# hyllios/CGAT

Measured on AMD Instinct MI355X. Metric: edges/sec through one CGAT attention layer (fwd+bwd), 1M-edge batch, higher is better.
Workload: dtype f32 storage / f16x3c (24-bit operands: exact h + l + t split, 3 fp16 + 3 six-bit matrix passes where built, six bf16 passes elsewhere; fp32 accumulate); 1 GPU; one GATConvNodes layer (H_Net update) fwd+bwd, 4167 crystals x 20 atoms x 12 nbrs per rank: N=83340, E=1000080, C=Ce=128, H=3, scalar attention; edges_per_rank=1000080, parallelism=dp1 (graphs sharded, gradient all-reduce)

## Files before the change

### cgat_amd/csrc/rowsdw.hip

```cpp
#include <string.h>

#include "common.h"
#include "kernels.h"
#include "mfma_bf16.h"

typedef float f32x16 __attribute__((ext_vector_type(16)));

template <int NX>
__device__ __forceinline__ void rows_dw128_body(const float* __restrict__ G, long ldg, const float* __restrict__ X1,
                                                long ldx1, const float* __restrict__ X2, long ldx2,
                                                float* __restrict__ o, int nbeg, int nend, float* red) {
  constexpr int U = 4;
  const int tid = threadIdx.x, lane = tid & 63, wave = tid >> 6;
  const int w = wave & 3, h = wave >> 2;
  const int l32 = lane & 31, hi = lane >> 5;
  const int nbatch = (nend - nbeg + 4 * U - 1) / (4 * U);

  f32x16 acc[NX][4];
#pragma unroll
  for (int k = 0; k < NX; ++k)
#pragma unroll
    for (int j = 0; j < 4; ++j)
#pragma unroll
      for (int t = 0; t < 16; ++t) acc[k][j][t] = 0.f;
  float cs = 0.f;

  float ga[3][U];
  float4 xa[3][U], xb[3][NX > 1 ? U : 1];
#define DW_LOAD(buf_, b_)                                                                     \
  {                                                                                           \
    _Pragma("unroll") for (int u = 0; u < U; ++u) {                                           \
      const int row = nbeg + 2 * U * (2 * (b_) + h) + 2 * u + hi;                             \
      const bool ok = row < nend;                                                             \
      const long rr = ok ? row : nbeg;                                                        \
      const float g = G[rr * ldg + 4 * l32 + w];                                              \
      const float4 x = *reinterpret_cast<const float4*>(X1 + rr * ldx1 + 4 * l32);            \
      ga[buf_][u] = ok ? g : 0.f;                                                             \
      xa[buf_][u] = x;                                                                        \
      if constexpr (NX > 1) xb[buf_][u] = *reinterpret_cast<const float4*>(X2 + rr * ldx2 + 4 * l32); \
    }                                                                                         \
  }
#define DW_MFMA(buf_)                                                                         \
  {                                                                                           \
    _Pragma("unroll") for (int u = 0; u < U; ++u) {                                           \
      const float a = ga[buf_][u];                                                            \
      cs += a;                                                                                \
      acc[0][0] = __builtin_amdgcn_mfma_f32_32x32x2f32(a, xa[buf_][u].x, acc[0][0], 0, 0, 0); \
      acc[0][1] = __builtin_amdgcn_mfma_f32_32x32x2f32(a, xa[buf_][u].y, acc[0][1], 0, 0, 0); \
      acc[0][2] = __builtin_amdgcn_mfma_f32_32x32x2f32(a, xa[buf_][u].z, acc[0][2], 0, 0, 0); \
      acc[0][3] = __builtin_amdgcn_mfma_f32_32x32x2f32(a, xa[buf_][u].w, acc[0][3], 0, 0, 0); \
      if constexpr (NX > 1) {                                                                 \
        acc[NX - 1][0] = __builtin_amdgcn_mfma_f32_32x32x2f32(a, xb[buf_][u].x, acc[NX - 1][0], 0, 0, 0); \
        acc[NX - 1][1] = __builtin_amdgcn_mfma_f32_32x32x2f32(a, xb[buf_][u].y, acc[NX - 1][1], 0, 0, 0); \
        acc[NX - 1][2] = __builtin_amdgcn_mfma_f32_32x32x2f32(a, xb[buf_][u].z, acc[NX - 1][2], 0, 0, 0); \
        acc[NX - 1][3] = __builtin_amdgcn_mfma_f32_32x32x2f32(a, xb[buf_][u].w, acc[NX - 1][3], 0, 0, 0); \
      }                                                                                       \
    }                                                                                         \
  }
  DW_LOAD(0, 0);
  DW_LOAD(1, 1);
  for (int b = 0; b < nbatch; b += 3) {
    DW_LOAD(2, b + 2);
    DW_MFMA(0);
    if (b + 1 < nbatch) {
      DW_LOAD(0, b + 3);
      DW_MFMA(1);
    }
    if (b + 2 < nbatch) {
      DW_LOAD(1, b + 4);
      DW_MFMA(2);
    }
  }
#undef DW_LOAD
#undef DW_MFMA
  cs += __shfl_xor(cs, 32);
  if (h == 1) {
#pragma unroll
    for (int k = 0; k < NX; ++k)
#pragma unroll
      for (int t = 0; t < 16; ++t) {
        const int m = (t & 3) + 8 * (t >> 2) + 4 * hi;
        *reinterpret_cast<float4*>(&red[(k * 128 + 4 * m + w) * 128 + 4 * l32]) =
            make_float4(acc[k][0][t], acc[k][1][t], acc[k][2][t], acc[k][3][t]);
      }
    if (hi == 0) red[NX * 128 * 128 + 4 * l32 + w] = cs;
  }
  __syncthreads();
  if (h == 0) {
#pragma unroll
    for (int k = 0; k < NX; ++k)
#pragma unroll
      for (int t = 0; t < 16; ++t) {
        const int m = (t & 3) + 8 * (t >> 2) + 4 * hi;
        const int idx = (k * 128 + 4 * m + w) * 128 + 4 * l32;
        const float4 r = *reinterpret_cast<const float4*>(&red[idx]);
        *reinterpret_cast<float4*>(o + idx) =
            make_float4(acc[k][0][t] + r.x, acc[k][1][t] + r.y, acc[k][2][t] + r.z, acc[k][3][t] + r.w);
      }
    if (hi == 0) o[NX * 128 * 128 + 4 * l32 + w] = cs + red[NX * 128 * 128 + 4 * l32 + w];
  }
}

template <int NX>
__global__ __launch_bounds__(512, 1) void rows_dw128_kernel(const float* __restrict__ G, long ldg,
                                                            const float* __restrict__ X1, long ldx1,
                                                            const float* __restrict__ X2, long ldx2,
                                                            float* __restrict__ slab, int rows, int rows_per_wg) {
  constexpr int SLAB = NX * 128 * 128 + 128;
  extern __shared__ float red[];
  const int nbeg = blockIdx.x * rows_per_wg;
  rows_dw128_body<NX>(G, ldg, X1, ldx1, X2, ldx2, slab + (long)blockIdx.x * SLAB, nbeg, min(rows, nbeg + rows_per_wg), red);
}

__global__ __launch_bounds__(512, 1) void rows_dw128_batch_kernel(DwBatchDesc d, float* __restrict__ slab) {
  extern __shared__ float red[];
  const int item = blockIdx.x / d.splits, sp = blockIdx.x - item * d.splits;
  const float* G = d.it[item].G;
  const float* X = d.it[item].X;
  const int nbeg = sp * d.rows_per_unit;
  rows_dw128_body<1>(G, d.ldg, X, d.ldx, X, d.ldx, slab + (long)blockIdx.x * (16384 + 128), nbeg,
                     min(d.rows, nbeg + d.rows_per_unit), red);
}
#define DWS_PITCH 80
#define DWS_IMG (128 * DWS_PITCH)
__global__ __launch_bounds__(512, 1) void rows_dw128_split_batch_kernel(DwBatchDesc d, float* __restrict__ slab) {
  extern __shared__ __attribute__((aligned(16))) unsigned char lds[];
  const int item = blockIdx.x / d.splits, sp = blockIdx.x - item * d.splits;
  const float* G = d.it[item].G;
  const float* X = d.it[item].X;
  const int nbeg = sp * d.rows_per_unit, nend = min(d.rows, nbeg + d.rows_per_unit);
  float* o = slab + (long)blockIdx.x * (16384 + 128);
  const int tid = threadIdx.x, lane = tid & 63, wave = tid >> 6;
  const int opnd = tid >> 8, m = tid & 127, half = (tid >> 7) & 1;
  const float* src = opnd ? X : G;
  const long ld = opnd ? d.ldx : d.ldg;
  unsigned char* wr_base = lds + (size_t)opnd * 3 * DWS_IMG + (size_t)m * DWS_PITCH + half * 32;
  const int wo = wave & 3, wi = wave >> 2;
  const int n16 = lane & 15, kg = lane >> 4;
  const unsigned char* rdA = lds + (size_t)(32 * wo + n16) * DWS_PITCH + kg * 16;
  const unsigned char* rdB = lds + (size_t)3 * DWS_IMG + (size_t)(64 * wi + n16) * DWS_PITCH + kg * 16;

  f32x4 accp[8], accn[8];
#pragma unroll
  for (int i = 0; i < 8; ++i) { accp[i] = f32x4{0.f, 0.f, 0.f, 0.f}; accn[i] = f32x4{0.f, 0.f, 0.f, 0.f}; }
  float cs = 0.f;
  const int nsteps = (nend - nbeg + 31) / 32;

  float va[16], vb[16];
#define DWS_LOAD(V_, s_)                                                                     \
  {                                                                                          \
    _Pragma("unroll") for (int u = 0; u < 16; ++u) {                                         \
      const int row = nbeg + 32 * (s_) + 16 * half + u;                                      \
      const bool ok = row < nend;                                                            \
      const float t = src[(long)(ok ? row : nend - 1) * ld + m];                             \
      V_[u] = (ok || opnd) ? t : 0.f;                                                        \
    }                                                                                        \
  }
#define DWS_STEP(V_, s_, ACC_, NEG_)                                                         \
  {                                                                                          \
    {                                                                                        \
      float w[16];                                                                           \
      _Pragma("unroll") for (int u = 0; u < 16; ++u) {                                       \
        if (!opnd) cs += V_[u];                                                              \
        w[u] = (NEG_ && !opnd) ? -V_[u] : V_[u];                                             \
      }                                                                                      \
      unsigned char* wp = wr_base + (size_t)((s_) & 1) * 6 * DWS_IMG;                        \
      _Pragma("unroll") for (int h8 = 0; h8 < 2; ++h8) {                                     \
        const float v8[8] = {w[8 * h8], w[8 * h8 + 1], w[8 * h8 + 2], w[8 * h8 + 3],         \
                             w[8 * h8 + 4], w[8 * h8 + 5], w[8 * h8 + 6], w[8 * h8 + 7]};    \
        bf16x8 q1, q2, q3;                                                                   \
        split3_x8(v8, q1, q2, q3);                                                           \
        *reinterpret_cast<bf16x8*>(wp + 16 * h8) = q1;                                       \
        *reinterpret_cast<bf16x8*>(wp + DWS_IMG + 16 * h8) = q2;                             \
        *reinterpret_cast<bf16x8*>(wp + 2 * DWS_IMG + 16 * h8) = q3;                         \
      }                                                                                      \
    }                                                                                        \
    DWS_LOAD(V_, (s_) + 2)    \
     \
    asm volatile("s_waitcnt lgkmcnt(0)" ::: "memory");                                       \
    __builtin_amdgcn_s_barrier();                                                            \
    asm volatile("" ::: "memory");                                                           \
    {                                                                                        \
      const unsigned char* pa = rdA + (size_t)((s_) & 1) * 6 * DWS_IMG;                      \
      const unsigned char* pb = rdB + (size_t)((s_) & 1) * 6 * DWS_IMG;                      \
      bf16x8 a1[2], a2[2], a3[2];                                                            \
      _Pragma("unroll") for (int ob = 0; ob < 2; ++ob) {                                     \
        a1[ob] = *reinterpret_cast<const bf16x8*>(pa + (size_t)16 * ob * DWS_PITCH);         \
        a2[ob] = *reinterpret_cast<const bf16x8*>(pa + DWS_IMG + (size_t)16 * ob * DWS_PITCH);      \
        a3[ob] = *reinterpret_cast<const bf16x8*>(pa + 2 * DWS_IMG + (size_t)16 * ob * DWS_PITCH);  \
      }                                                                                      \
      _Pragma("unroll") for (int ib = 0; ib < 4; ++ib) {                                     \
        const bf16x8 b1 = *reinterpret_cast<const bf16x8*>(pb + (size_t)16 * ib * DWS_PITCH);               \
        const bf16x8 b2 = *reinterpret_cast<const bf16x8*>(pb + DWS_IMG + (size_t)16 * ib * DWS_PITCH);     \
        const bf16x8 b3 = *reinterpret_cast<const bf16x8*>(pb + 2 * DWS_IMG + (size_t)16 * ib * DWS_PITCH); \
        _Pragma("unroll") for (int ob = 0; ob < 2; ++ob) {                                   \
          f32x4 c = ACC_[4 * ob + ib];                                                       \
          c = mma16<false>(a3[ob], b1, c);                         \
          c = mma16<false>(a1[ob], b3, c);                                                   \
          c = mma16<false>(a2[ob], b2, c);                                                   \
          c = mma16<false>(a2[ob], b1, c);                                                   \
          c = mma16<false>(a1[ob], b2, c);                                                   \
          c = mma16<false>(a1[ob], b1, c);                                                   \
          ACC_[4 * ob + ib] = c;                                                             \
        }                                                                                    \
      }                                                                                      \
    }                                                                                        \
  }
  DWS_LOAD(va, 0)
  DWS_LOAD(vb, 1)
  for (int s = 0; s < nsteps; s += 2) {
    DWS_STEP(va, s, accp, false)
    DWS_STEP(vb, s + 1, accn, true)
  }
#undef DWS_LOAD
#undef DWS_STEP
#pragma unroll
  for (int ob = 0; ob < 2; ++ob)
#pragma unroll
    for (int ib = 0; ib < 4; ++ib)
#pragma unroll
      for (int t = 0; t < 4; ++t) {
        const int orow = 32 * wo + 16 * ob + 4 * kg + t, icol = 64 * wi + 16 * ib + n16;
        float r = accp[4 * ob + ib][t] - accn[4 * ob + ib][t];
        asm volatile("" : "+v"(r));
        o[orow * 128 + icol] = r;
      }
  __syncthreads();
  float* red = reinterpret_cast<float*>(lds);
  if (!opnd && half == 1) red[m] = cs;
  __syncthreads();
  if (!opnd && half == 0) o[16384 + m] = cs + red[m];
}

__global__ __launch_bounds__(256) void rows_dw128_reduce_batch_kernel(const float* __restrict__ slab, DwBatchDesc d) {
  __shared__ float part[8][32];
  const int item = blockIdx.y;
  const int o = threadIdx.x & 31, zg = threadIdx.x >> 5;
  const long total = 16384 + 128;
  const long i = (long)blockIdx.x * 32 + o;
  const float* sl = slab + (long)item * d.splits * total;
  const int per = (d.splits + 7) / 8;
  const int z0 = zg * per, z1 = min(d.splits, z0 + per);
  float s = 0.f;
  if (i < total)
    for (int z = z0; z < z1; ++z) s += sl[(long)z * total + i];
  part[zg][o] = s;
  __syncthreads();
  if (zg != 0 || i >= total) return;
  s = part[0][o];
#pragma unroll
  for (int g = 1; g < 8; ++g) s += part[g][o];
  if (i < 16384) d.it[item].out[(i >> 7) * d.ldo + (i & 127)] = s;
  else if (d.it[item].bsum) d.it[item].bsum[i - 16384] = s;
}

__global__ __launch_bounds__(256) void rows_dw128_reduce_kernel(const float* __restrict__ slab, int splits, int nx,
                                                                float* __restrict__ out1, long ldo1,
                                                                float* __restrict__ out2, long ldo2,
                                                                float* __restrict__ bsum) {
  __shared__ float part[8][32];
  const int o = threadIdx.x & 31, zg = threadIdx.x >> 5;
  const long total = (long)nx * 16384 + 128, stride = total;
  const long i = (long)blockIdx.x * 32 + o;
  const int per = (splits + 7) / 8;
  const int z0 = zg * per, z1 = min(splits, z0 + per);
  float s = 0.f;
  if (i < total)
    for (int z = z0; z < z1; ++z) s += slab[(long)z * stride + i];
  part[zg][o] = s;
  __syncthreads();
  if (zg != 0 || i >= total) return;
  s = part[0][o];
#pragma unroll
  for (int g = 1; g < 8; ++g) s += part[g][o];
  if (i < 16384) out1[(i >> 7) * ldo1 + (i & 127)] = s;
  else if (nx > 1 && i < 32768) out2[((i - 16384) >> 7) * ldo2 + (i & 127)] = s;
  else if (bsum) bsum[i - (long)nx * 16384] = s;
}

int rows_dw128_batch_launch(DwBatchDesc d, void* ws, size_t ws_bytes, hipStream_t stream);
static int dw_rows_per_wg(int rows) {
  int rps = cdiv(cdiv(rows, 256), 16) * 16;
  return rps < 16 ? 16 : rps;
}
bool rows_dw128_fast(const float* G, long ldg, const float* X1, long ldx1, const float* X2, long ldx2) {
  return (ldg % 4) == 0 && (ldx1 % 4) == 0 && (((uintptr_t)G) & 15) == 0 && (((uintptr_t)X1) & 15) == 0 &&
         (!X2 || ((ldx2 % 4) == 0 && (((uintptr_t)X2) & 15) == 0));
}
size_t rows_dw128_batch_ws_bytes(int n_items, int rows);
size_t rows_dw128_ws_bytes(int rows, int nx) {
  const int splits = cdiv(rows, dw_rows_per_wg(rows));
  size_t b = ws_round((size_t)splits * ((size_t)nx * 16384 + 128), 4);
  if (nx == 1) {
    const size_t c = rows_dw128_batch_ws_bytes(1, rows);
    if (c > b) b = c;
  }
  return b;
}
int rows_dw128_launch(const float* G, long ldg, const float* X1, long ldx1, float* out1, long ldo1, const float* X2,
                      long ldx2, float* out2, long ldo2, float* bsum, int rows, void* ws, size_t ws_bytes,
                      hipStream_t stream) {
  const int nx = X2 ? 2 : 1;
  if (rows <= 0) {
    for (int o = 0; o < 128; ++o) {
      CGAT_TRY(fill_launch(out1 + o * ldo1, 0.f, 128, stream));
      if (X2) CGAT_TRY(fill_launch(out2 + o * ldo2, 0.f, 128, stream));
    }
    if (bsum) CGAT_TRY(fill_launch(bsum, 0.f, 128, stream));
    return CGAT_OK;
  }
  const size_t need = rows_dw128_ws_bytes(rows, nx);
  if (!ws || ws_bytes < need) {
    cgat_set_error("rows_dw128: workspace too small (%zu < %zu)", ws_bytes, need);
    return CGAT_ERR_WORKSPACE;
  }
  if (nx == 1 && mode_split()) {
    DwBatchDesc b;
    memset(&b, 0, sizeof(b));
    b.n = 1; b.rows = rows; b.ldg = ldg; b.ldx = ldx1; b.ldo = ldo1;
    b.it[0] = {G, X1, out1, bsum};
    return rows_dw128_batch_launch(b, ws, ws_bytes, stream);
  }
  const int rps = dw_rows_per_wg(rows), splits = cdiv(rows, rps);
  const size_t lds = ((size_t)nx * 16384 + 128) * sizeof(float);
  {
    CGAT_PROF("rows_dw", stream);
    if (nx == 2) {
      static bool attr = false;
      if (!attr) {
        CGAT_HIP(hipFuncSetAttribute((const void*)rows_dw128_kernel<2>, hipFuncAttributeMaxDynamicSharedMemorySize, (int)lds));
        attr = true;
      }
      hipLaunchKernelGGL(rows_dw128_kernel<2>, dim3(splits), dim3(512), lds, stream, G, ldg, X1, ldx1, X2, ldx2,
                         (float*)ws, rows, rps);
    } else {
      static bool attr = false;
      if (!attr) {
        CGAT_HIP(hipFuncSetAttribute((const void*)rows_dw128_kernel<1>, hipFuncAttributeMaxDynamicSharedMemorySize, (int)lds));
        attr = true;
      }
      hipLaunchKernelGGL(rows_dw128_kernel<1>, dim3(splits), dim3(512), lds, stream, G, ldg, X1, ldx1, X1, ldx1,
                         (float*)ws, rows, rps);
    }
    CGAT_LAUNCH_CHECK();
  }
  const long total = (long)nx * 16384 + 128;
  hipLaunchKernelGGL(rows_dw128_reduce_kernel, dim3(cdiv(total, 32)), dim3(256), 0, stream, (const float*)ws, splits, nx,
                     out1, ldo1, out2, ldo2, bsum);
  CGAT_LAUNCH_CHECK();
  return CGAT_OK;
}

static int dw_batch_splits(int n_items, int rows) {
  int sp = 256 / (n_items > 0 ? n_items : 1);
  const int most = cdiv(rows, 64);
  if (sp > most) sp = most;
  return sp < 1 ? 1 : sp;
}
size_t rows_dw128_batch_ws_bytes(int n_items, int rows) {
  if (n_items < 1) n_items = 1;
  const long most = cdiv(rows > 0 ? rows : 1, 64);
  long units = n_items > 256 ? n_items : 256;
  if (units > (long)n_items * most) units = (long)n_items * most;
  return ws_round((size_t)units * (16384 + 128), 4);
}
bool rows_dw128_batch_fast(const DwBatchDesc& d) {
  if (d.n < 1 || d.n > DW_BATCH_MAX || d.rows < 1) return false;
  for (int i = 0; i < d.n; ++i)
    if (!rows_dw128_fast(d.it[i].G, d.ldg, d.it[i].X, d.ldx, nullptr, 0)) return false;
  return true;
}
int rows_dw128_batch_launch(DwBatchDesc d, void* ws, size_t ws_bytes, hipStream_t stream) {
  if (!rows_dw128_batch_fast(d)) {
    cgat_set_error("rows_dw128_batch: not the fast shape (n = %d, rows = %d)", d.n, d.rows);
    return CGAT_ERR_UNSUPPORTED;
  }
  const size_t need = ws_round((size_t)d.n * dw_batch_splits(d.n, d.rows) * (16384 + 128), 4);
  if (!ws || ws_bytes < need) {
    cgat_set_error("rows_dw128_batch: workspace too small (%zu < %zu)", ws_bytes, need);
    return CGAT_ERR_WORKSPACE;
  }
  const bool split_form = mode_split();
  d.splits = dw_batch_splits(d.n, d.rows);
  d.rows_per_unit = cdiv(cdiv(d.rows, d.splits), 32) * 32;
  d.splits = cdiv(d.rows, d.rows_per_unit);
  const size_t lds = (16384 + 128) * sizeof(float);
  if (split_form) {
    CGAT_PROF("rows_dw", stream);
    const size_t lds2 = (size_t)2 * 2 * 3 * DWS_IMG;
    static bool attr2 = false;
    if (!attr2) {
      CGAT_HIP(hipFuncSetAttribute((const void*)rows_dw128_split_batch_kernel, hipFuncAttributeMaxDynamicSharedMemorySize, (int)lds2));
      attr2 = true;
    }
    hipLaunchKernelGGL(rows_dw128_split_batch_kernel, dim3(d.n * d.splits), dim3(512), lds2, stream, d, (float*)ws);
    CGAT_LAUNCH_CHECK();
  } else {
    CGAT_PROF("rows_dw", stream);
    static bool attr = false;
    if (!attr) {
      CGAT_HIP(hipFuncSetAttribute((const void*)rows_dw128_batch_kernel, hipFuncAttributeMaxDynamicSharedMemorySize, (int)lds));
      attr = true;
    }
    hipLaunchKernelGGL(rows_dw128_batch_kernel, dim3(d.n * d.splits), dim3(512), lds, stream, d, (float*)ws);
    CGAT_LAUNCH_CHECK();
  }
  hipLaunchKernelGGL(rows_dw128_reduce_batch_kernel, dim3(cdiv(16384 + 128, 32), d.n), dim3(256), 0, stream,
                     (const float*)ws, d);
  CGAT_LAUNCH_CHECK();
  return CGAT_OK;
}
```

Before: 37.30 million edges/s.

## Deepen rows_dw split kernel pipeline, interleaving loads and splits with MFMA

Restructures the split-bf16 weight-gradient kernel so global loads for step s+5 and the bf16x3 split/LDS writes for step s+1 are interleaved with the MFMA loop of step s. The prefetch depth grows from two to four register buffers, and the kernel now has one barrier per step. It also adds a sign flip by XOR and a pairwise split helper. This hides global-load latency and split ALU work behind matrix ops, at the cost of more registers and odd-step padding handled through dws_steps rounding.

```diff
diff --git a/cgat_amd/csrc/rowsdw.hip b/cgat_amd/csrc/rowsdw.hip
--- a/cgat_amd/csrc/rowsdw.hip
+++ b/cgat_amd/csrc/rowsdw.hip
@@ -3,6 +3,7 @@
 #include "common.h"
 #include "kernels.h"
 #include "mfma_bf16.h"
+#include "rowsdw_map.h"
 
 typedef float f32x16 __attribute__((ext_vector_type(16)));
 
@@ -121,8 +122,6 @@
   rows_dw128_body<1>(G, d.ldg, X, d.ldx, X, d.ldx, slab + (long)blockIdx.x * (16384 + 128), nbeg,
                      min(d.rows, nbeg + d.rows_per_unit), red);
 }
-#define DWS_PITCH 80
-#define DWS_IMG (128 * DWS_PITCH)
 __global__ __launch_bounds__(512, 1) void rows_dw128_split_batch_kernel(DwBatchDesc d, float* __restrict__ slab) {
   extern __shared__ __attribute__((aligned(16))) unsigned char lds[];
   const int item = blockIdx.x / d.splits, sp = blockIdx.x - item * d.splits;
@@ -130,89 +129,120 @@
   const float* X = d.it[item].X;
   const int nbeg = sp * d.rows_per_unit, nend = min(d.rows, nbeg + d.rows_per_unit);
   float* o = slab + (long)blockIdx.x * (16384 + 128);
-  const int tid = threadIdx.x, lane = tid & 63, wave = tid >> 6;
-  const int opnd = tid >> 8, m = tid & 127, half = (tid >> 7) & 1;
+  const int tid = threadIdx.x, lane = tid & 63;
+  const int wave = __builtin_amdgcn_readfirstlane(tid >> 6);
+  const DwsLoader ldr = dws_loader(64 * wave);
+  const int opnd = ldr.opnd, half = ldr.half;
+  const unsigned m = (unsigned)dws_loader(tid).m;
   const float* src = opnd ? X : G;
   const long ld = opnd ? d.ldx : d.ldg;
-  unsigned char* wr_base = lds + (size_t)opnd * 3 * DWS_IMG + (size_t)m * DWS_PITCH + half * 32;
-  const int wo = wave & 3, wi = wave >> 2;
+  unsigned char* wr_base = lds + dws_write_off(0, opnd, 0, m, half, 0);
   const int n16 = lane & 15, kg = lane >> 4;
-  const unsigned char* rdA = lds + (size_t)(32 * wo + n16) * DWS_PITCH + kg * 16;
-  const unsigned char* rdB = lds + (size_t)3 * DWS_IMG + (size_t)(64 * wi + n16) * DWS_PITCH + kg * 16;
+  const unsigned char* rdA = lds + dws_frag_off(0, 0, 0, dws_col_a(wave, 0, n16), kg);
+  const unsigned char* rdB = lds + dws_frag_off(0, 1, 0, dws_col_b(wave, 0, n16), kg);
 
   f32x4 accp[8], accn[8];
 #pragma unroll
   for (int i = 0; i < 8; ++i) { accp[i] = f32x4{0.f, 0.f, 0.f, 0.f}; accn[i] = f32x4{0.f, 0.f, 0.f, 0.f}; }
   float cs = 0.f;
-  const int nsteps = (nend - nbeg + 31) / 32;
-
-  float va[16], vb[16];
-#define DWS_LOAD(V_, s_)                                                                     \
+  const unsigned negmask = opnd ? 0u : 0x80000000u;
+  const int nsteps = dws_steps(nbeg, nend);
+
+  float va[16], vb[16], vc[16], vd[16];
+  unsigned w1[4], w2[4], w3[4];
+#define DWS_LOAD4(V_, s_, u0_)                                                               \
   {                                                                                          \
-    _Pragma("unroll") for (int u = 0; u < 16; ++u) {                                         \
-      const int row = nbeg + 32 * (s_) + 16 * half + u;                                      \
-      const bool ok = row < nend;                                                            \
-      const float t = src[(long)(ok ? row : nend - 1) * ld + m];                             \
-      V_[u] = (ok || opnd) ? t : 0.f;                                                        \
+    _Pragma("unroll") for (int u = (u0_); u < (u0_) + 4; ++u) {                              \
+      V_[u] = src[(long)dws_src_row(dws_load_row(nbeg, (s_), half, u), nend) * ld + m];      \
     }                                                                                        \
   }
-#define DWS_STEP(V_, s_, ACC_, NEG_)                                                         \
+#define DWS_SPLIT4(V_, s_, NEG_, p_)                                                         \
   {                                                                                          \
-    {                                                                                        \
-      float w[16];                                                                           \
-      _Pragma("unroll") for (int u = 0; u < 16; ++u) {                                       \
-        if (!opnd) cs += V_[u];                                                              \
-        w[u] = (NEG_ && !opnd) ? -V_[u] : V_[u];                                             \
-      }                                                                                      \
-      unsigned char* wp = wr_base + (size_t)((s_) & 1) * 6 * DWS_IMG;                        \
-      _Pragma("unroll") for (int h8 = 0; h8 < 2; ++h8) {                                     \
-        const float v8[8] = {w[8 * h8], w[8 * h8 + 1], w[8 * h8 + 2], w[8 * h8 + 3],         \
-                             w[8 * h8 + 4], w[8 * h8 + 5], w[8 * h8 + 6], w[8 * h8 + 7]};    \
-        bf16x8 q1, q2, q3;                                                                   \
-        split3_x8(v8, q1, q2, q3);                                                           \
-        *reinterpret_cast<bf16x8*>(wp + 16 * h8) = q1;                                       \
-        *reinterpret_cast<bf16x8*>(wp + DWS_IMG + 16 * h8) = q2;                             \
-        *reinterpret_cast<bf16x8*>(wp + 2 * DWS_IMG + 16 * h8) = q3;                         \
-      }                                                                                      \
+    float w[4];                                                                              \
+    _Pragma("unroll") for (int u = 0; u < 4; ++u) {                                          \
+      const bool ok = dws_load_row(nbeg, (s_), half, 4 * (p_) + u) < nend;                   \
+      const float t = (ok || opnd) ? V_[4 * (p_) + u] : 0.f;    \
+      cs += t;                                             \
+      w[u] = __builtin_bit_cast(float, __builtin_bit_cast(unsigned, t) ^ ((NEG_) ? negmask : 0u)); \
     }                                                                                        \
-    DWS_LOAD(V_, (s_) + 2)    \
-     \
+    split3_pair(w[0], w[1], w1[2 * ((p_) & 1)], w2[2 * ((p_) & 1)], w3[2 * ((p_) & 1)]);     \
+    split3_pair(w[2], w[3], w1[2 * ((p_) & 1) + 1], w2[2 * ((p_) & 1) + 1], w3[2 * ((p_) & 1) + 1]); \
+    if ((p_) & 1) {                                                                          \
+      unsigned char* wp = wr_base + (size_t)((s_) & 1) * DWS_BUF + 16 * ((p_) >> 1);         \
+      *reinterpret_cast<uint4*>(wp) = make_uint4(w1[0], w1[1], w1[2], w1[3]);                \
+      *reinterpret_cast<uint4*>(wp + DWS_IMG) = make_uint4(w2[0], w2[1], w2[2], w2[3]);      \
+      *reinterpret_cast<uint4*>(wp + 2 * DWS_IMG) = make_uint4(w3[0], w3[1], w3[2], w3[3]);  \
+    }                                                                                        \
+  }
+#define DWS_READ_B(ib_)                                                                      \
+  {                                                                                          \
+    b1 = *reinterpret_cast<const bf16x8*>(pb + (size_t)16 * (ib_) * DWS_PITCH);              \
+    b2 = *reinterpret_cast<const bf16x8*>(pb + DWS_IMG + (size_t)16 * (ib_) * DWS_PITCH);    \
+    b3 = *reinterpret_cast<const bf16x8*>(pb + 2 * DWS_IMG + (size_t)16 * (ib_) * DWS_PITCH); \
+  }
+#define DWS_BARRIER()                                                                        \
+  {                                                                                          \
     asm volatile("s_waitcnt lgkmcnt(0)" ::: "memory");                                       \
     __builtin_amdgcn_s_barrier();                                                            \
     asm volatile("" ::: "memory");                                                           \
-    {                                                                                        \
-      const unsigned char* pa = rdA + (size_t)((s_) & 1) * 6 * DWS_IMG;                      \
-      const unsigned char* pb = rdB + (size_t)((s_) & 1) * 6 * DWS_IMG;                      \
-      bf16x8 a1[2], a2[2], a3[2];                                                            \
+  }
+#define DWS_STEP(s_, ACC_, VN_, NEGN_)                                                       \
+  {                                                                                          \
+    const unsigned char* pa = rdA + (size_t)((s_) & 1) * DWS_BUF;                            \
+    const unsigned char* pb = rdB + (size_t)((s_) & 1) * DWS_BUF;                            \
+    bf16x8 a1[2], a2[2], a3[2];                                                              \
+    _Pragma("unroll") for (int ob = 0; ob < 2; ++ob) {                                       \
+      a1[ob] = *reinterpret_cast<const bf16x8*>(pa + (size_t)16 * ob * DWS_PITCH);           \
+      a2[ob] = *reinterpret_cast<const bf16x8*>(pa + DWS_IMG + (size_t)16 * ob * DWS_PITCH); \
+      a3[ob] = *reinterpret_cast<const bf16x8*>(pa + 2 * DWS_IMG + (size_t)16 * ob * DWS_PITCH); \
+    }                                                                                        \
+    _Pragma("unroll") for (int ib = 0; ib < 4; ++ib) {                                       \
+      bf16x8 b1, b2, b3;                                                                     \
+      DWS_READ_B(ib)                                                                         \
+      DWS_SPLIT4(VN_, (s_) + 1, NEGN_, ib)                                                   \
+      DWS_LOAD4(VN_, (s_) + 5, 4 * ib)                                                       \
       _Pragma("unroll") for (int ob = 0; ob < 2; ++ob) {                                     \
-        a1[ob] = *reinterpret_cast<const bf16x8*>(pa + (size_t)16 * ob * DWS_PITCH);         \
-        a2[ob] = *reinterpret_cast<const bf16x8*>(pa + DWS_IMG + (size_t)16 * ob * DWS_PITCH);      \
-        a3[ob] = *reinterpret_cast<const bf16x8*>(pa + 2 * DWS_IMG + (size_t)16 * ob * DWS_PITCH);  \
-      }                                                                                      \
-      _Pragma("unroll") for (int ib = 0; ib < 4; ++ib) {                                     \
-        const bf16x8 b1 = *reinterpret_cast<const bf16x8*>(pb + (size_t)16 * ib * DWS_PITCH);               \
-        const bf16x8 b2 = *reinterpret_cast<const bf16x8*>(pb + DWS_IMG + (size_t)16 * ib * DWS_PITCH);     \
-        const bf16x8 b3 = *reinterpret_cast<const bf16x8*>(pb + 2 * DWS_IMG + (size_t)16 * ib * DWS_PITCH); \
-        _Pragma("unroll") for (int ob = 0; ob < 2; ++ob) {                                   \
-          f32x4 c = ACC_[4 * ob + ib];                                                       \
-          c = mma16<false>(a3[ob], b1, c);                         \
-          c = mma16<false>(a1[ob], b3, c);                                                   \
-          c = mma16<false>(a2[ob], b2, c);                                                   \
-          c = mma16<false>(a2[ob], b1, c);                                                   \
-          c = mma16<false>(a1[ob], b2, c);                                                   \
-          c = mma16<false>(a1[ob], b1, c);                                                   \
-          ACC_[4 * ob + ib] = c;                                                             \
-        }                                                                                    \
+        f32x4 c = ACC_[4 * ob + ib];                                                         \
+        c = mma16<false>(a3[ob], b1, c);                           \
+        c = mma16<false>(a1[ob], b3, c);                                                     \
+        c = mma16<false>(a2[ob], b2, c);                                                     \
+        c = mma16<false>(a2[ob], b1, c);                                                     \
+        c = mma16<false>(a1[ob], b2, c);                                                     \
+        c = mma16<false>(a1[ob], b1, c);                                                     \
+        ACC_[4 * ob + ib] = c;                                                               \
       }                                                                                      \
     }                                                                                        \
-  }
-  DWS_LOAD(va, 0)
-  DWS_LOAD(vb, 1)
-  for (int s = 0; s < nsteps; s += 2) {
-    DWS_STEP(va, s, accp, false)
-    DWS_STEP(vb, s + 1, accn, true)
-  }
-#undef DWS_LOAD
+    DWS_BARRIER()                                                                            \
+  }
+#pragma unroll
+  for (int p = 0; p < 4; ++p) DWS_LOAD4(va, 0, 4 * p)
+#pragma unroll
+  for (int p = 0; p < 4; ++p) DWS_LOAD4(vb, 1, 4 * p)
+#pragma unroll
+  for (int p = 0; p < 4; ++p) DWS_LOAD4(vc, 2, 4 * p)
+#pragma unroll
+  for (int p = 0; p < 4; ++p) DWS_LOAD4(vd, 3, 4 * p)
+#pragma unroll
+  for (int p = 0; p < 4; ++p) {
+    DWS_SPLIT4(va, 0, false, p)
+    DWS_LOAD4(va, 4, 4 * p)
+  }
+  DWS_BARRIER()
+  int s = 0;
+  for (; s + 4 <= nsteps; s += 4) {
+    DWS_STEP(s, accp, vb, true)
+    DWS_STEP(s + 1, accn, vc, false)
+    DWS_STEP(s + 2, accp, vd, true)
+    DWS_STEP(s + 3, accn, va, false)
+  }
+  if (s < nsteps) {
+    DWS_STEP(s, accp, vb, true)
+    DWS_STEP(s + 1, accn, vc, false)
+  }
+#undef DWS_LOAD4
+#undef DWS_SPLIT4
+#undef DWS_READ_B
+#undef DWS_BARRIER
 #undef DWS_STEP
 #pragma unroll
   for (int ob = 0; ob < 2; ++ob)
@@ -220,12 +250,11 @@
     for (int ib = 0; ib < 4; ++ib)
 #pragma unroll
       for (int t = 0; t < 4; ++t) {
-        const int orow = 32 * wo + 16 * ob + 4 * kg + t, icol = 64 * wi + 16 * ib + n16;
+        const int orow = dws_col_a(wave, ob, 0) + 4 * kg + t, icol = dws_col_b(wave, ib, n16);
         float r = accp[4 * ob + ib][t] - accn[4 * ob + ib][t];
         asm volatile("" : "+v"(r));
         o[orow * 128 + icol] = r;
       }
-  __syncthreads();
   float* red = reinterpret_cast<float*>(lds);
   if (!opnd && half == 1) red[m] = cs;
   __syncthreads();
@@ -351,12 +380,6 @@
   return CGAT_OK;
 }
 
-static int dw_batch_splits(int n_items, int rows) {
-  int sp = 256 / (n_items > 0 ? n_items : 1);
-  const int most = cdiv(rows, 64);
-  if (sp > most) sp = most;
-  return sp < 1 ? 1 : sp;
-}
 size_t rows_dw128_batch_ws_bytes(int n_items, int rows) {
   if (n_items < 1) n_items = 1;
   const long most = cdiv(rows > 0 ? rows : 1, 64);
@@ -381,13 +404,13 @@
     return CGAT_ERR_WORKSPACE;
   }
   const bool split_form = mode_split();
-  d.splits = dw_batch_splits(d.n, d.rows);
-  d.rows_per_unit = cdiv(cdiv(d.rows, d.splits), 32) * 32;
-  d.splits = cdiv(d.rows, d.rows_per_unit);
+  const DwPartition part = dw_batch_partition(d.n, d.rows);
+  d.splits = part.splits;
+  d.rows_per_unit = part.rows_per_unit;
   const size_t lds = (16384 + 128) * sizeof(float);
   if (split_form) {
     CGAT_PROF("rows_dw", stream);
-    const size_t lds2 = (size_t)2 * 2 * 3 * DWS_IMG;
+    const size_t lds2 = DWS_LDS_BYTES;
     static bool attr2 = false;
     if (!attr2) {
       CGAT_HIP(hipFuncSetAttribute((const void*)rows_dw128_split_batch_kernel, hipFuncAttributeMaxDynamicSharedMemorySize, (int)lds2));
diff --git a/cgat_amd/csrc/rowsdw_map.h b/cgat_amd/csrc/rowsdw_map.h
--- /dev/null
+++ b/cgat_amd/csrc/rowsdw_map.h
@@ -0,0 +1,53 @@
+#pragma once
+
+#ifdef __HIPCC__
+#define DWS_HD __host__ __device__ __forceinline__
+#else
+#define DWS_HD static inline
+#endif
+
+#define DWS_ROWS 32
+#define DWS_PITCH 80
+#define DWS_IMG (128 * DWS_PITCH)
+#define DWS_BUF (6 * DWS_IMG)
+#define DWS_LDS_BYTES (2 * DWS_BUF)
+
+DWS_HD int dw_batch_splits(int n_items, int rows) {
+  int sp = 256 / (n_items > 0 ? n_items : 1);
+  const int most = (rows + 63) / 64;
+  if (sp > most) sp = most;
+  return sp < 1 ? 1 : sp;
+}
+struct DwPartition {
+  int splits, rows_per_unit;
+};
+DWS_HD DwPartition dw_batch_partition(int n_items, int rows) {
+  DwPartition p;
+  p.splits = dw_batch_splits(n_items, rows);
+  p.rows_per_unit = (((rows + p.splits - 1) / p.splits + DWS_ROWS - 1) / DWS_ROWS) * DWS_ROWS;
+  p.splits = (rows + p.rows_per_unit - 1) / p.rows_per_unit;
+  return p;
+}
+DWS_HD int dws_steps(int nbeg, int nend) { return (((nend - nbeg + DWS_ROWS - 1) / DWS_ROWS) + 1) & ~1; }
+
+struct DwsLoader {
+  int opnd, m, half;
+};
+DWS_HD DwsLoader dws_loader(int tid) {
+  DwsLoader l;
+  l.opnd = tid >> 8;
+  l.m = tid & 127;
+  l.half = (tid >> 7) & 1;
+  return l;
+}
+DWS_HD int dws_load_row(int nbeg, int s, int half, int u) { return nbeg + DWS_ROWS * s + 16 * half + u; }
+DWS_HD int dws_src_row(int row, int nend) { return row < nend ? row : nend - 1; }
+DWS_HD unsigned dws_write_off(int s, int opnd, int plane, int m, int half, int h8) {
+  return (unsigned)((s & 1) * DWS_BUF + (opnd * 3 + plane) * DWS_IMG + m * DWS_PITCH + half * 32 + 16 * h8);
+}
+
+DWS_HD int dws_col_a(int wave, int ob, int n16) { return 32 * (wave & 3) + 16 * ob + n16; }
+DWS_HD int dws_col_b(int wave, int ib, int n16) { return 64 * (wave >> 2) + 16 * ib + n16; }
+DWS_HD unsigned dws_frag_off(int s, int opnd, int plane, int col, int kg) {
+  return (unsigned)((s & 1) * DWS_BUF + (opnd * 3 + plane) * DWS_IMG + col * DWS_PITCH + kg * 16);
+}
```

Measured after the change: 37.42 million edges/s (median of 6 runs). About the same (+0.3%).
